# mpetri/ans-large-alphabet

Measured on AMD Instinct MI355X. Metric: encode+decode Mints/s (uint32), bit-exact vs CPU reference per block, higher is better.
Workload: dtype u32 symbols; ANS state carried as an exact f64 (integers below 2^53) in the encoder, u64 in the decoder; 1 GPU; ANSfold-1 on 268435456 uint32 per GPU, zipf20s1.2, blocks of 16384 ints, restart every 1024; codec=ANSfold-1, ints_per_gpu=268435456, distribution=zipf20s1.2, block_ints=16384, ckpt_interval=1024, seed=1234, multi_gpu=single GPU

## Files before the change

ans_large_alphabet_amd/csrc/ansx.hip:

```cpp
#include "../../include/ansx.h"

#include <hip/hip_runtime.h>
#include <dlfcn.h>
#include <rccl/rccl.h>

#include <algorithm>
#include <array>
#include <cmath>
#include <cstdio>
#include <cstdlib>
#include <cstring>
#include <deque>
#include <functional>
#include <map>
#include <set>
#include <string>
#include <vector>

#include "ansx_kernels.h"
#include "ansx_rfold.h"
#include "ansx_model.h"
#include "ansx_fastmodel.h"
#include "ansx_gen.h"
#include "ansx_pa.h"
#include "ansx_intsparse.h"
#include "ansx_ranges.h"
#include "ansx_batch.h"

namespace {

struct DevBuf {
    void* p = nullptr;
    size_t cap = 0;
};

struct ProfRec {
    std::string name;
    hipEvent_t e0, e1;
};

struct Layout {
    u64 index_off, ckoff_off, ckstate_off, hint_off, payload_off;
};

}

struct ansx_ctx {
    u32 num_cus = 256;
    int device = 0;
    hipStream_t stream = nullptr;
    int last_hip = 0;
    bool profile = false;
    std::vector<ProfRec> recs;
    std::map<std::string, std::pair<double, u64>> acc;
    std::vector<std::string> order;
    DevBuf pre_work;
    DevBuf hist, hterm, sortF, sortSym, attS, prevS, attMeta, blk, table, tab32, scratch, misc, mapped, mostfreq,
        stage_in, stage_out, dec_s2s, dec_cum, dec_info, plain, rf_tmp, log2lut, pa_alpha, pa_info, pairs, lg2i, sizes, nearlist, force;
    DevBuf rng_plan, rng_cont, rng_list;
    DevBuf rng_dev;
    DevBuf bat_hdr;
    u8* rng_pin = nullptr;
    size_t rng_pin_cap = 0;
    u32* h_pin = nullptr;
    std::map<u64, u32> ns_hint;
    std::map<u64, u32> rf_hint;
    std::map<std::array<u64, 4>, ansx_container_header> hdr_cache;
    std::deque<std::array<u64, 4>> hdr_order;
    std::map<u32, DevBuf> geo;
    DevBuf geo_big;
    u32 geo_big_cap = 0;
    int last_gather_ranks = 0;
    std::set<u64> wide_hint;
    std::map<u64, u32> t_hint;
    const u32* cur_force = nullptr;
    const u32* cur_src = nullptr;
    bool used_pc = false;
    bool used_fast = false;
    u32 cur_nt = 0;
    u32 cur_rf_slots = 0;
    u32 cur_pa_distinct = 0;
    std::set<u64> int_sparse_hint;
    bool cur_int_sparse = false;
    u32 sp_retries = 0;
    bool sp_full_lds = false;
    ansx_encode_stats last = {};
    struct {
        bool table16_fixup = false;
        bool encode_gtab16 = false;
        bool parse_generic = false;
        bool parse_win = false;
        bool parse_fast = false;
        bool decode_table = false;
        bool no_stream_lds = false;
        int decode_mode = 0;
        u32 parse_stage_words = 0;
        bool model_fused = false;
        bool model_sync = false;
        bool use_pc = false;
        u32 pc_b_pairs = 2;
        u32 test_sp_bits = 0;
        bool fin_one_wave = false;
        bool no_big_geo = false;
        bool no_pc_auto = false;
        bool encode_mode2 = false;
        bool force_pc = false;
        bool no_pc = false;
        int decode_small_ring = 0;
        int decode_pair = 0;
        u32 pair_lds_limit = 0;
        u32 wide_at = 16;
        bool wide_restart = false;
        u32 ns_hint = 0;
        u32 t_hint = 0;
        bool no_fast_model = false;
        double near_band = ANSX_NEAR_BAND;
        bool near_flip = false;
        u32 cand_chains = 0;
        double fast_guard = ANSX_FAST_GUARD;
        u32 batch_pass_blocks = 0;
    } dbg;
};

namespace {

#define HIPCHK(ctx, call)                                                                        \
    do {                                                                                         \
        hipError_t _e = (call);                                                                  \
        if (_e != hipSuccess) {                                                                  \
            (ctx)->last_hip = (int)_e;                                                           \
            return ANSX_ERR_HIP;                                                                 \
        }                                                                                        \
    } while (0)

int ensure(ansx_ctx* c, DevBuf& b, size_t bytes)
{
    if (bytes <= b.cap) return ANSX_OK;
    if (b.p) {
        hipError_t e = hipFree(b.p);
        b.p = nullptr;
        b.cap = 0;
        if (e != hipSuccess) {
// ... 16 lines not shown
    if (!c->profile) return;
    ProfRec r;
    r.name = name;
    (void)hipEventCreate(&r.e0);
    (void)hipEventCreate(&r.e1);
    (void)hipEventRecord(r.e0, s);
    c->recs.push_back(r);
}
void prof_end(ansx_ctx* c, hipStream_t s)
{
    if (!c->profile) return;
    (void)hipEventRecord(c->recs.back().e1, s);
}

#define LAUNCH(ctx, name, kern, grid, block, shmem, strm, ...)                                   \
    do {                                                                                         \
        prof_begin(ctx, name, strm);                                                             \
        hipLaunchKernelGGL(kern, dim3(grid), dim3(block), (shmem), strm, __VA_ARGS__);           \
        prof_end(ctx, strm);                                                                     \
        HIPCHK(ctx, hipGetLastError());                                                          \
    } while (0)

inline size_t rup(size_t v, size_t a) { return (v + a - 1) / a * a; }

size_t codec_nsp(int kind, u32 f) { return kind == ANSX_MSB ? 2048u : (kind == ANSX_INT ? 16384u : fold_NSP(f)); }

size_t block_bound(int kind, u32 f, size_t nb, bool pa = false)
{
    size_t hdr = kind == ANSX_RFOLD ? 4 + 4 * (size_t)fold_T(f) : 0;
    size_t nsp = codec_nsp(kind, f);
    if (pa) hdr += 8 + 4 * nb + 8;
    return hdr + 8 + 4 * nsp + 7 * nb + 32;
}

struct Plan {
    ansx_geo g;
    bool plain;
    Layout lay;
    u32 NSP;
    const ansx_blk_out* bout = nullptr;
    u64 bout_ints = 0;
};

Layout layout_of(const ansx_geo& g, bool plain)
{
    Layout L;
// ... 355 lines not shown
        && !c->dbg.encode_gtab16 && (u64)scr_stride * 16 < 0x7FFFFF00ull;
    c->used_fast = fast;
    if (fast && NSP > 4096 && !c->dbg.no_big_geo) {
        if (c->geo_big_cap < fcap_probe) {
            if ((rc = ensure(c, c->geo_big, ((size_t)fcap_probe * (fcap_probe + 1) / 2 + 8) * 8))) return rc;
            LAUNCH(c, "k_build_interp_geo", k_build_interp_geo, fcap_probe, 256, 0, s, fcap_probe, (uint2*)c->geo_big.p);
            c->geo_big_cap = fcap_probe;
        }
        geo = (const uint2*)c->geo_big.p;
    }
    if (fast) {
        if ((rc = ensure(c, c->pairs, (size_t)NB * NSP * 8))) return rc;
        if (!c->lg2i.p) {
            if ((rc = ensure(c, c->lg2i, (size_t)65536 * 8))) return rc;
            LAUNCH(c, "k_build_log2i_lut", k_build_log2i_lut, 256, 256, 0, s, (double*)c->lg2i.p);
        }
    }
    double* hterm = nullptr;
    if (h_deferred && !h_in_hist && !fast) {
        if ((rc = ensure(c, c->hterm, (size_t)NB * NSP * 8))) return rc;
        hterm = (double*)c->hterm.p;
    }
    const size_t hist_lds = !h_in_hist ? (size_t)NSP * 4 : (size_t)4 * (NSP + ANSX_HCOPY_PAD) * 4 + (fast ? 0 : (size_t)NSP * 8 + 80);
    if (NSP >= 8192u) {
        const size_t packed_lds = (size_t)NSP * 2;
        if (packed_lds > 48 * 1024)
            HIPCHK(c, hipFuncSetAttribute((const void*)k_fold_hist<true>, hipFuncAttributeMaxDynamicSharedMemorySize, (int)packed_lds));
        LAUNCH(c, "k_fold_hist", k_fold_hist<true>, (size_t)NB * cpb, 256, packed_lds, s, src, g, chunk, cpb, NSP, hist, hterm,
            fast ? 2u : 0u, blk, gflags, (g.kind == ANSX_INT && !g.pa) ? NSP : (1u << 30));
    } else {
        if (hist_lds > 48 * 1024)
            HIPCHK(c, hipFuncSetAttribute((const void*)k_fold_hist<false>, hipFuncAttributeMaxDynamicSharedMemorySize, (int)hist_lds));
        LAUNCH(c, "k_fold_hist", k_fold_hist<false>, (size_t)NB * cpb, 256, hist_lds, s, src, g, chunk, cpb, NSP, hist, hterm,
            (h_in_hist ? 1u : 0u) | (fast ? 2u : 0u), blk, gflags, (g.kind == ANSX_INT && !g.pa) ? NSP : (1u << 30));
    }
    const u32 nbig_cap = (u32)std::min<size_t>(NSP, (size_t)g.block_ints / ANSX_VMAX + 2);
    const u32 sort_cap = (optimistic && h_deferred) ? std::min<u32>(NSP, std::max<u32>(64u, (ns_cap + 7u) & ~7u)) : NSP;
    const bool sort16 = g.block_ints <= 65535u;
    size_t k2a_lds = (size_t)nbig_cap * 8 + (size_t)sort_cap * (sort16 ? 2 : 4) + (h_deferred ? 0 : 512 * 8);
    const bool sort_staged = k2a_lds <= 150 * 1024;
    if (!sort_staged) k2a_lds = (size_t)nbig_cap * 8 + (h_deferred ? 0 : 512 * 8);
    if (k2a_lds > 32 * 1024) {
        HIPCHK(c, hipFuncSetAttribute((const void*)k_sort_entropy<u16>, hipFuncAttributeMaxDynamicSharedMemorySize, (int)k2a_lds));
        HIPCHK(c, hipFuncSetAttribute((const void*)k_sort_entropy<u32>, hipFuncAttributeMaxDynamicSharedMemorySize, (int)k2a_lds));
    }
    if ((size_t)NSP * 8 + 64 > 48 * 1024 && (size_t)NSP * 8 + 64 <= 150 * 1024)
        HIPCHK(c, hipFuncSetAttribute((const void*)k_write_prelude<0>,
                      hipFuncAttributeMaxDynamicSharedMemorySize, (int)((size_t)NSP * 8 + 64)));
    if (!sort_staged)
        LAUNCH(c, "k_sort_entropy", (k_sort_entropy<u32, false>), NB, 64, k2a_lds, s, g, NSP, nbig_cap, h_deferred ? 1u : 0u, hist,
            (u32*)c->sortF.p, (u16*)c->sortSym.p, blk, sort_cap, fast ? (uint2*)c->pairs.p : (uint2*)nullptr, gflags);
    else if (sort16)
        LAUNCH(c, "k_sort_entropy", k_sort_entropy<u16>, NB, 64, k2a_lds, s, g, NSP, nbig_cap, h_deferred ? 1u : 0u, hist,
            (u32*)c->sortF.p, (u16*)c->sortSym.p, blk, sort_cap, fast ? (uint2*)c->pairs.p : (uint2*)nullptr, gflags);
    else
        LAUNCH(c, "k_sort_entropy", k_sort_entropy<u32>, NB, 64, k2a_lds, s, g, NSP, nbig_cap, h_deferred ? 1u : 0u, hist,
            (u32*)c->sortF.p, (u16*)c->sortSym.p, blk, sort_cap, fast ? (uint2*)c->pairs.p : (uint2*)nullptr, gflags);
    const u32 nbatch = 24 / ANSX_ATTEMPTS;
    u32 max_logM = 0, max_ns = 0;
    const bool test_fixup = c->dbg.table16_fixup;
    const u32 always16 = (!test_fixup && (NSP > 4096 || (u64)scr_stride * 16 >= 0x7FFFFF00ull || c->dbg.encode_gtab16)) ? 1u : 0u;
    u32* hints = (P.plain || (g.kind == ANSX_INT && !g.pa)) ? nullptr : (u32*)(d_out + P.lay.hint_off);
    if (fast) {
        const u32 bpw = 64u / NT;
        const u32 nch = c->dbg.cand_chains ? c->dbg.cand_chains : (((NB + bpw - 1) / bpw <= 4u * c->num_cus) ? 1u : 2u);
        const size_t cl = (size_t)ANSX_CAND_WAVES * nch * bpw * ANSX_CAND_ROW * 16;
        const u32 cwaves = (NB + nch * bpw - 1) / (nch * bpw);
#define ANSX_LAUNCH_CAND2(NT_, NCH_)                                                                                    \
    do {                                                                                                            \
        if (cl > 48 * 1024)                                                                                         \
            HIPCHK(c, hipFuncSetAttribute((const void*)k_candidates<NT_, NCH_>, hipFuncAttributeMaxDynamicSharedMemorySize, (int)cl)); \
        LAUNCH(c, "k_candidates", (k_candidates<NT_, NCH_>), (cwaves + ANSX_CAND_WAVES - 1) / ANSX_CAND_WAVES, 64 * ANSX_CAND_WAVES, cl, s, g, NSP, \
            (const uint2*)c->pairs.p, (const ansx_blk*)blk, (uint4*)c->attS.p, (u32*)c->attMeta.p);               \
    } while (0)
#define ANSX_LAUNCH_CAND(NT_)                                                                                           \
    do {                                                                                                            \
        if (nch == 1) ANSX_LAUNCH_CAND2(NT_, 1);                                                                    \
        else ANSX_LAUNCH_CAND2(NT_, 2);                                                                             \
    } while (0)
        switch (NT) {
        case 4: ANSX_LAUNCH_CAND(4); break;
        case 5: ANSX_LAUNCH_CAND(5); break;
        case 6: ANSX_LAUNCH_CAND(6); break;
        case 7: ANSX_LAUNCH_CAND(7); break;
        default: ANSX_LAUNCH_CAND(8); break;
        }
#undef ANSX_LAUNCH_CAND
#undef ANSX_LAUNCH_CAND2
        const u32 fcap = std::min<u32>(NSP, std::max<u32>(64u, (ns_cap + 15u) & ~15u));
        const bool fin_generic = NSP > 4096;
        const size_t fl = (size_t)fcap * (fin_generic ? 8 : 12) + 64;
#define ANSX_LAUNCH_FIN(IPT_, NTC_)                                                                                    \
    do {                                                                                                            \
        if (fl > 48 * 1024)                                                                                         \
            HIPCHK(c, hipFuncSetAttribute((const void*)k_model_finish<IPT_, NTC_>, hipFuncAttributeMaxDynamicSharedMemorySize, (int)fl)); \
        LAUNCH(c, "k_model_finish", (k_model_finish<IPT_, NTC_>), NB, 256, fl, s, g, NSP, NT, (const uint2*)c->pairs.p, (const uint4*)c->attS.p, \
            (const u32*)c->attMeta.p, blk, (u32*)c->tab32.p, (u8*)c->scratch.p, (u64)scr_stride, mostfreq, hints, gflags, fcap, c->dbg.fast_guard, (const double*)c->lg2i.p, geo, \
            fin_generic ? hist : (u32*)nullptr); \
    } while (0)
        if (NSP <= 1024 && c->dbg.fin_one_wave) {
            if (NT <= 5) {
                LAUNCH(c, "k_model_finish", (k_model_finish<16, 5, 64>), NB, 64, fl, s, g, NSP, NT, (const uint2*)c->pairs.p, (const uint4*)c->attS.p,
                    (const u32*)c->attMeta.p, blk, (u32*)c->tab32.p, (u8*)c->scratch.p, (u64)scr_stride, mostfreq, hints, gflags, fcap, c->dbg.fast_guard, (const double*)c->lg2i.p, geo,
                    (u32*)nullptr);
            } else {
                LAUNCH(c, "k_model_finish", (k_model_finish<16, 8, 64>), NB, 64, fl, s, g, NSP, NT, (const uint2*)c->pairs.p, (const uint4*)c->attS.p,
                    (const u32*)c->attMeta.p, blk, (u32*)c->tab32.p, (u8*)c->scratch.p, (u64)scr_stride, mostfreq, hints, gflags, fcap, c->dbg.fast_guard, (const double*)c->lg2i.p, geo,
                    (u32*)nullptr);
            }
        } else if (NSP <= 1024) {
            ANSX_LAUNCH_FIN(4, 8);
        } else if (NSP > 4096) {
            if (NT <= 5) ANSX_LAUNCH_FIN(0, 5);
            else ANSX_LAUNCH_FIN(0, 8);
        } else {
            if (NT <= 5) ANSX_LAUNCH_FIN(16, 5);
            else ANSX_LAUNCH_FIN(16, 8);
        }
#undef ANSX_LAUNCH_FIN
        max_logM = 16;
        max_ns = ns_cap;
    }
    for (u32 batch = 0; batch < (fast ? 0u : nbatch); batch++) {
        if (batch) HIPCHK(c, hipMemsetAsync(&gflags[ANSX_G_PAD], 0, 4, s));
        LAUNCH(c, "k_scale_attempts", k_scale_attempts, ((size_t)NB * ANSX_ATTEMPTS + 255) / 256, 256,
            0, s, g, NSP, batch, hist, (const u32*)c->sortF.p, (const u16*)c->sortSym.p, blk,
            (u16*)c->attS.p, (u32*)c->attMeta.p, (const double*)hterm, (const ansx_log2_ent*)c->log2lut.p,
            g.block_ints <= 65535u ? 1u : 0u);
        LAUNCH(c, "k_select_model", k_select_model, NB, 64, 0, s, g, NSP, batch, hist,
            (const u16*)c->attS.p, (const u32*)c->attMeta.p, (u16*)c->prevS.p, blk,
            (ansx_enc_entry*)c->table.p, (u32*)c->tab32.p, gflags, batch == nbatch - 1 ? 1u : 0u, always16,
            (u32*)c->nearlist.p, c->cur_force, c->dbg.near_band, c->dbg.near_flip ? 1u : 0u);
        if (optimistic) {
            max_logM = 16;
            max_ns = ns_cap;
            break;
        }
        HIPCHK(c, hipMemcpyAsync(c->h_pin, c->misc.p, 16, hipMemcpyDeviceToHost, s));
        HIPCHK(c, hipStreamSynchronize(s));
        int st0 = flags_to_status(c->h_pin[ANSX_G_ERR]);
        if (st0) return st0;
        max_logM = c->h_pin[ANSX_G_MAXLOGM];
// ... 1251 lines not shown
    if (hipGetDeviceCount(&ndev) != hipSuccess || ndev == 0) return ANSX_ERR_NO_DEVICE;
    if (device < 0) {
        if (hipGetDevice(&device) != hipSuccess) return ANSX_ERR_NO_DEVICE;
    }
    if (device >= ndev) return ANSX_ERR_ARG;
    if (hipSetDevice(device) != hipSuccess) return ANSX_ERR_NO_DEVICE;
    hipDeviceProp_t prop;
    if (hipGetDeviceProperties(&prop, device) != hipSuccess) return ANSX_ERR_NO_DEVICE;
    if (strncmp(prop.gcnArchName, "gfx950", 6) != 0) return ANSX_ERR_NO_DEVICE;
    ansx_ctx* c = new ansx_ctx();
    c->device = device;
    c->num_cus = prop.multiProcessorCount > 0 ? (u32)prop.multiProcessorCount : 256u;
    if (hipStreamCreateWithFlags(&c->stream, hipStreamDefault) != hipSuccess) {
        delete c;
        return ANSX_ERR_HIP;
    }
    if (hipHostMalloc((void**)&c->h_pin, 4096, hipHostMallocDefault) != hipSuccess) {
        (void)hipStreamDestroy(c->stream);
        delete c;
        return ANSX_ERR_HIP;
    }
    static const char* const names[] = { "ANSX_TEST_TABLE16_FIXUP", "ANSX_ENCODE_GTAB16", "ANSX_PARSE_GENERIC", "ANSX_PARSE_WIN", "ANSX_PARSE_FAST",
        "ANSX_DECODE_TABLE", "ANSX_NO_STREAM_LDS", "ANSX_DECODE_MODE", "ANSX_PARSE_STAGE_WORDS", "ANSX_MODEL_FUSED", "ANSX_MODEL_SYNC", "ANSX_NS_HINT", "ANSX_T_HINT", "ANSX_NO_FAST_MODEL", "ANSX_FAST_GUARD", "ANSX_CAND_CHAINS", "ANSX_NEAR_BAND", "ANSX_TEST_NEAR_FLIP", "ANSX_WIDE_RESTART", "ANSX_TEST_WIDE_AT",
        "ANSX_BATCH_PASS_BLOCKS" };
    for (const char* nm : names)
        if (const char* v = getenv(nm)) (void)ansx_debug_set(c, nm, v);
    *out = c;
    return ANSX_OK;
}

int ansx_last_encode_stats(const ansx_ctx* c, ansx_encode_stats* out)
{
    if (!c || !out) return ANSX_ERR_ARG;
    *out = c->last;
#ifdef ANSX_STAMPS
    {
        static unsigned long long h[16 * 256 + 16];
        if (hipMemcpyFromSymbol(h, HIP_SYMBOL(g_stamps), sizeof(h)) == hipSuccess) {
            double acc[16] = {};
            int nn = 0;
#ifdef ANSX_STAMPS_RF
            const int last = 8;
#else
            const int last = 10;
#endif
            for (int w = 0; w < 256; w++) {
                if (!h[w * 16] || !h[w * 16 + last]) continue;
// ... 57 lines not shown
    else if (!strcmp(name, "ANSX_PC_B_PAIRS")) c->dbg.pc_b_pairs = (value && value[0] == '1') ? 1u : 2u;
    else if (!strcmp(name, "ANSX_ENCODE_MODE2")) c->dbg.encode_mode2 = on;
    else if (!strcmp(name, "ANSX_DECODE_SMALL_RING"))
        c->dbg.decode_small_ring = !value ? 0 : !strcmp(value, "never") ? 1 : !strcmp(value, "always") ? 2 : 0;
    else if (!strcmp(name, "ANSX_DECODE_PAIR"))
        c->dbg.decode_pair = !value ? 0 : !strcmp(value, "never") ? 1 : !strcmp(value, "always") ? 2 : 0;
    else if (!strcmp(name, "ANSX_DECODE_PAIR_LDS")) c->dbg.pair_lds_limit = (value && value[0]) ? (u32)strtoul(value, nullptr, 10) : 0u;
    else if (!strcmp(name, "ANSX_FORGET_HINTS")) {
        c->ns_hint.clear();
        c->rf_hint.clear();
        c->t_hint.clear();
        c->wide_hint.clear();
        c->hdr_cache.clear();
        c->hdr_order.clear();
    }
    else if (!strcmp(name, "ANSX_TEST_WIDE_AT")) {
        const u32 v = (value && value[0]) ? (u32)strtoul(value, nullptr, 10) : 16u;
        if (v > 16) return ANSX_ERR_ARG;
        c->dbg.wide_at = v;
    }
    else if (!strcmp(name, "ANSX_NEAR_BAND")) c->dbg.near_band = (value && value[0]) ? strtod(value, nullptr) : ANSX_NEAR_BAND;
    else if (!strcmp(name, "ANSX_TEST_NEAR_FLIP")) c->dbg.near_flip = on;
    else if (!strcmp(name, "ANSX_BATCH_PASS_BLOCKS")) c->dbg.batch_pass_blocks = (value && value[0]) ? (u32)strtoul(value, nullptr, 10) : 0u;
    else if (!strcmp(name, "ANSX_CAND_CHAINS")) {
        const u32 v = value ? (u32)strtoul(value, nullptr, 10) : 0u;
        if (v > 2) return ANSX_ERR_ARG;
        c->dbg.cand_chains = v;
    } else if (!strcmp(name, "ANSX_FAST_GUARD")) c->dbg.fast_guard = (value && value[0]) ? strtod(value, nullptr) : ANSX_FAST_GUARD;
    else return ANSX_ERR_ARG;
    return ANSX_OK;
}

void ansx_destroy(ansx_ctx* c)
{
    if (!c) return;
    (void)hipSetDevice(c->device);
    (void)hipStreamSynchronize(c->stream);
    DevBuf* bufs[] = { &c->pre_work, &c->hist, &c->hterm, &c->sortF, &c->sortSym, &c->attS, &c->prevS, &c->attMeta, &c->blk,
        &c->table, &c->tab32, &c->scratch, &c->misc, &c->mapped, &c->mostfreq, &c->stage_in, &c->stage_out,
        &c->dec_s2s, &c->dec_cum, &c->dec_info, &c->plain, &c->rf_tmp, &c->log2lut, &c->pa_alpha, &c->pa_info, &c->pairs, &c->lg2i, &c->sizes, &c->nearlist, &c->force, &c->geo_big,
        &c->rng_plan, &c->rng_cont, &c->rng_list, &c->rng_dev, &c->bat_hdr };
    for (DevBuf* b : bufs)
        if (b->p) (void)hipFree(b->p);
    for (auto& kv : c->geo)
        if (kv.second.p) (void)hipFree(kv.second.p);
    for (auto& r : c->recs) {
        (void)hipEventDestroy(r.e0);
        (void)hipEventDestroy(r.e1);
    }
    if (c->h_pin) (void)hipHostFree(c->h_pin);
    if (c->rng_pin) (void)hipHostFree(c->rng_pin);
    (void)hipStreamDestroy(c->stream);
    delete c;
}

const char* ansx_strerror(int st)
{
    switch (st) {
    case ANSX_OK: return "ok";
    case ANSX_ERR_ARG: return "invalid argument";
// ... 460 lines not shown
```

ans_large_alphabet_amd/csrc/ansx_fastmodel.h:

```cpp
#pragma once

#include "ansx_kernels.h"

#ifdef ANSX_STAMPS_RF
#undef STAMP
#define STAMP(i) do { } while (0)
#endif

#define ANSX_FAST_GUARD 1e-9
#define ANSX_CAND_SL 64u
#define ANSX_CAND_ROW (ANSX_CAND_SL + 1u)
#define ANSX_CAND_MAXBPW 16u
#define ANSX_FIN_LUT 512u

__global__ void k_build_log2i_lut(double* __restrict__ lut)
{
    const u32 i = blockIdx.x * 256 + threadIdx.x;
    if (i < 65536u) lut[i] = i ? ansx_log2_portable((double)i) : 0.0;
}

__device__ __forceinline__ double ansx_rcp_int31(double b)
{
    const double y0 = __builtin_amdgcn_rcp(b);
    const double y1 = __builtin_fma(__builtin_fma(-b, y0, 1.0), y0, y0);
    return __builtin_fma(__builtin_fma(-b, y1, 1.0), y1, y1);
}

ANSX_HD u64 srank_chunk(u32 NSP, u32 NT, u32 b, u32 batch, u32 t) { return ((u64)b * (NSP / 8u) + batch) * NT + t; }

#define ANSX_CAND_WAVES 4u
template <u32 NT, u32 NCH>
__global__ __launch_bounds__(64 * ANSX_CAND_WAVES) void k_candidates(ansx_geo g, u32 NSP,
    const uint2* __restrict__ pairs, const ansx_blk* __restrict__ blk, uint4* __restrict__ srank,
    u32* __restrict__ attMeta)
{
    extern __shared__ double2 cand_lds_all[];
    const u32 lane = threadIdx.x & 63u, wv = threadIdx.x >> 6;
    constexpr u32 BPW = 64u / NT;
    constexpr u32 rows = NCH * BPW;
    double2* const cand_lds = cand_lds_all + wv * rows * ANSX_CAND_ROW;
    const u32 bl = lane / NT, t = lane - bl * NT;
    const u32 wb0 = (u32)__builtin_amdgcn_readfirstlane((int)((blockIdx.x * ANSX_CAND_WAVES + wv) * rows));
    if (wb0 >= g.nblocks) return;
    u32 bb[NCH], sigma[NCH], sh[NCH];
    bool live[NCH];
    double Md[NCH], fsd[NCH], mx[NCH];
    uint4* sp[NCH];
    const double2* row[NCH];
    u32 wsig = 0;
#pragma unroll
    for (u32 c = 0; c < NCH; c++) {
        bb[c] = wb0 + c * BPW + bl;
        live[c] = bl < BPW && bb[c] < g.nblocks;
        sigma[c] = 0, sh[c] = 0;
        double nd = 1.0;
        if (live[c]) {
            const ansx_blk* B = &blk[bb[c]];
            sigma[c] = B->sigma;
            sh[c] = B->m0_log2 + t;
            nd = (double)B->n;
        }
        wsig = sigma[c] > wsig ? sigma[c] : wsig;
        const bool dead = sh[c] > 31;
        Md[c] = dead ? -1.0 : (double)((u64)1 << (dead ? 0u : sh[c]));
        fsd[c] = nd;
        mx[c] = 0.0;
        sp[c] = srank + srank_chunk(NSP, NT, live[c] ? bb[c] : wb0, 0u, t);
        row[c] = cand_lds + (c * BPW + (bl < BPW ? bl : BPW - 1u)) * ANSX_CAND_ROW;
    }
    wsig = wave_max(wsig);
    constexpr u32 NITER = rows * (ANSX_CAND_SL / 64u);
    uint2 nxt[NITER];
    const u32 last_b = g.nblocks - 1u;
    auto fetch = [&](u32 c0) {
#pragma unroll
        for (u32 k = 0; k < NITER; k++) {
            const u32 i = k * 64u + lane;
            u32 b2 = wb0 + i / ANSX_CAND_SL;
            b2 = b2 < last_b ? b2 : last_b;
            u32 j = c0 + (i % ANSX_CAND_SL);
            j = j < NSP ? j : NSP - 1u;
            nxt[k] = pairs[(u64)b2 * NSP + j];
        }
    };
    auto commit = [&]() {
#pragma unroll
        for (u32 k = 0; k < NITER; k++) {
            const u32 i = k * 64u + lane;
            const u32 rem = nxt[k].y ? nxt[k].y : 1u;
            cand_lds[(i / ANSX_CAND_SL) * ANSX_CAND_ROW + (i % ANSX_CAND_SL)] =
                double2{ (double)(nxt[k].x & 0xFFFFu), ansx_rcp_int31((double)rem) };
        }
    };
    auto step = [&](u32 c, const double2 e) -> u32 {
        const double q = Md[c] * e.y;
        const double r = __builtin_fma(-q, fsd[c], Md[c]);
// ... 95 lines not shown
#ifdef ANSX_STAMPS
        t_loop += wall_clock64() - t_a;
#endif
    }
#ifdef ANSX_STAMPS
    if (threadIdx.x == 0 && blockIdx.x < 256) {
        g_stamps[blockIdx.x * 16 + 12] = t_commit;
        g_stamps[blockIdx.x * 16 + 13] = t_loop;
        g_stamps[blockIdx.x * 16 + 14] = wall_clock64() - tc0;
    }
#endif
#pragma unroll
    for (u32 c = 0; c < NCH; c++)
        if (live[c])
            *(uint2*)(attMeta + ((u64)bb[c] * ANSX_ATTEMPTS + t) * 4) =
                make_uint2((Md[c] == 0.0) ? 1u : 0u, mx[c] >= 4294967295.0 ? 0xFFFFFFFFu : (u32)mx[c]);
}

template <int IPT, int NTC, int NTH = 256>
__global__ __launch_bounds__(NTH) void k_model_finish(ansx_geo g, u32 NSP, u32 NT, const uint2* __restrict__ pairs,
    const uint4* __restrict__ srank, const u32* __restrict__ attMeta, ansx_blk* __restrict__ blk,
    u32* __restrict__ tab32, u8* __restrict__ scratch, u64 scr_stride, const u32* __restrict__ mostfreq,
    u32* __restrict__ hints, u32* __restrict__ gflags, u32 cap, double guard, const double* __restrict__ lg2i,
    const uint2* __restrict__ geo, u32* __restrict__ incbuf = nullptr)
{
    static_assert(IPT % 4 == 0, "table rows are written 16 bytes at a time");
    static_assert(ANSX_FIN_LUT == 512 && (NTH == 256 || NTH == 64), "two table entries per thread (eight in the one-wave form)");
    static_assert(NTH == 256 || (IPT > 4), "the one-wave form takes every candidate in every lane");
    static_assert(NTC >= 4 && NTC <= (int)ANSX_ATTEMPTS, "candidates per block");
    extern __shared__ u32 lds32[];
    __shared__ u32 sh_part[8];
    __shared__ double lut[ANSX_FIN_LUT];
    __shared__ double wpart[ANSX_ATTEMPTS][4];
    __shared__ double wsum[ANSX_ATTEMPTS];
    const u32 tid = threadIdx.x, lane = tid & 63u, wv = tid >> 6;
    const u32 b = blockIdx.x;
    ansx_blk* B = &blk[b];
    u32* off = lds32;
    u32* bits = lds32 + cap;
    const bool inc_hbm = IPT == 0 && incbuf != nullptr;
    u32* inc = inc_hbm ? incbuf + (u64)b * NSP : lds32 + 2 * cap;
    const u32 dump = inc_hbm ? cap + 8u : 2u * cap + 8u;
    u32* frq = bits;
    STAMP(0);
    const u32 ns = B->max_sym + 1;
    const u32 sigma = B->sigma;
    const double thr = B->thr;
    const u32 m0 = B->m0_log2;
    const double nd = (double)B->n;
    uint2 mt[ANSX_ATTEMPTS];
#pragma unroll
    for (u32 t = 0; t < ANSX_ATTEMPTS; t++) mt[t] = t < NT ? *(const uint2*)(attMeta + ((u64)b * ANSX_ATTEMPTS + t) * 4) : make_uint2(0u, 0u);
    double2 l2[256 / NTH];
#pragma unroll
    for (int i = 0; i < 256 / NTH; i++) l2[i] = *(const double2*)(lg2i + 2 * (tid + NTH * i));
    const uint2* prow = pairs + (u64)b * NSP;
    auto load_fs = [&](u32 c, u32 (&fs)[8]) {
        const uint2* pp = prow + (u64)c * 8u;
        const uint4 a0 = *(const uint4*)pp, a1 = *(const uint4*)(pp + 2), a2 = *(const uint4*)(pp + 4), a3 = *(const uint4*)(pp + 6);
// ... 243 lines not shown
```

ans_large_alphabet_amd/csrc/ansx_kernels.h:

```cpp
#pragma once

#include <type_traits>

#include "ansx_dev.h"

#ifdef ANSX_STAMPS
__device__ unsigned long long g_stamps[16 * 256 + 16];
#define STAMP(i) do { if (threadIdx.x == 0 && blockIdx.x % 61 == 7 && blockIdx.x / 61 < 256) g_stamps[(blockIdx.x / 61) * 16 + (i)] = wall_clock64(); } while (0)
#else
#define STAMP(i) do { } while (0)
#endif
#ifdef ANSX_STAMPS_RF
#define STAMP_RF(i) STAMP(i)
#else
#define STAMP_RF(i) do { } while (0)
#endif

struct ansx_blk {
    u32 n;
    u32 max_sym;
    u32 sigma;
    u32 m0_log2;
    double H;
    double thr;
// ... 39 lines not shown
struct ansx_zero4 {
    uint4* p[4];
    u64 n16[4];
};
__global__ __launch_bounds__(256) void k_begin_encode(ansx_zero4 Z)
{
    const u64 stride = (u64)gridDim.x * 256;
    const uint4 z = make_uint4(0u, 0u, 0u, 0u);
#pragma unroll
    for (int r = 0; r < 4; r++)
        for (u64 i = (u64)blockIdx.x * 256 + threadIdx.x; i < Z.n16[r]; i += stride) Z.p[r][i] = z;
}

#define ANSX_HCOPY_PAD 8u
typedef u32 ansx_u32x4 __attribute__((ext_vector_type(4)));
__device__ __forceinline__ uint4 ld16_stream(const uint4* p)
{
    const ansx_u32x4 v = __builtin_nontemporal_load((const ansx_u32x4*)p);
    return make_uint4(v.x, v.y, v.z, v.w);
}
template <bool PACKED>
__global__ __launch_bounds__(256) void k_fold_hist(const u32* __restrict__ in, ansx_geo g,
    u32 chunk, u32 cpb, u32 NSP, u32* __restrict__ hist, double* __restrict__ hterm, u32 sum_mode,
    ansx_blk* __restrict__ blk, u32* __restrict__ gflags, u32 value_limit)
{
    const u32 sum_here = sum_mode & 1u;
    const bool tree_sum = (sum_mode & 2u) != 0;
    extern __shared__ u32 lds_hist[];
    const u32 tid = threadIdx.x;
    const u32 b = blockIdx.x / cpb, c = blockIdx.x % cpb;
    const u32 nb = geo_block_n(g, b);
    const u64 start = (u64)c * chunk;
    if (start >= nb) return;
    const u32 len = (u32)((nb - start) < chunk ? (nb - start) : chunk);
    const u32* src = in + (u64)b * g.block_ints + start;
    const u32 cstride = sum_here ? NSP + ANSX_HCOPY_PAD : 0;
    const u32 hwords = sum_here ? 4 * cstride : (PACKED ? NSP / 2 : NSP);
    auto hcount = [&](u32 sy) -> u32 {
        if constexpr (PACKED) return (lds_hist[sy >> 1] >> (16u * (sy & 1u))) & 0xFFFFu;
        else return lds_hist[sy];
    };
    for (u32 s = tid; s < hwords; s += 256) lds_hist[s] = 0;
    u32* const aux = lds_hist + hwords;
    if (sum_here && !tree_sum && tid < 17) aux[2 * NSP + tid] = 0;
    u32* const my_hist = lds_hist + (tid & 3) * cstride;
    __syncthreads();
    const ansx_map mp = g.map;
    const bool ident = g.kind == 3;
    u32 lmax = 0, bad = 0;
    auto take = [&](u32 x) {
        bad |= (x >= value_limit) ? 1u : 0u;
        u32 k = map_nbytes(mp, x);
        u32 s = map_sym(mp, x, k);
// ... 98 lines not shown
        }
    } else {
        for (u32 s = tid; s < NSP; s += 256) {
            u32 v = hcount(s);
            if (v) atomicAdd(&h[s], v);
        }
    }
    lmax = wave_max(lmax);
    bad = wave_or(bad);
    if ((tid & 63) == 0) {
        atomicMax(&blk[b].max_sym, lmax);
        if (bad) atomicOr(&gflags[ANSX_G_ERR], 1u << 6 );
    }
}

#define ANSX_VMAX 256u
#define ANSX_MASKV 256u

__device__ __forceinline__ void wave_lds_sync() { asm volatile("s_waitcnt lgkmcnt(0)" ::: "memory"); }

template <typename HT, bool STAGED = true>
__global__ __launch_bounds__(64) void k_sort_entropy(ansx_geo g, u32 NSP, u32 nbig_cap, u32 h_deferred,
    const u32* __restrict__ hist, u32* __restrict__ sortF, u16* __restrict__ sortSym,
    ansx_blk* __restrict__ blk, u32 cap, uint2* __restrict__ pairs, u32* __restrict__ gflags)
{
    extern __shared__ u64 lds_k2a[];
    __shared__ u32 cnt[ANSX_VMAX];
    __shared__ u16 cnt0[ANSX_VMAX];
    __shared__ unsigned long long vmask[ANSX_MASKV];
    __shared__ u32 wadj[ANSX_VMAX];
    __shared__ u32 sh_nbig;
    u64* big_keys = lds_k2a;
    HT* hrow = (HT*)(lds_k2a + nbig_cap);
    double* terms = (double*)(hrow + (STAGED ? cap : 0u));
    const u32 lane = threadIdx.x;
    const u32 b = blockIdx.x;
    const u32* h = hist + (u64)b * NSP;
    constexpr u32 SORT_PRE = 10;
    u32 hp[SORT_PRE];
#pragma unroll
    for (u32 r = 0; r < SORT_PRE; r++) hp[r] = r * 64 + lane < NSP ? h[r * 64 + lane] : 0u;
    const u32 ns = blk[b].max_sym + 1;
    auto hget = [&](u32 sy) -> u32 {
        if constexpr (STAGED) return hrow[sy];
        else return h[sy];
    };
    if (STAGED && ns > cap) {
        if (lane == 0) {
            blk[b].status = 9;
            blk[b].resolved = 1;
            atomicOr(&gflags[ANSX_G_ERR], 1u << ANSX_G_VIOL_BIT);
        }
        return;
    }
    u32* oF = sortF + (u64)b * NSP;
    u16* oS = sortSym + (u64)b * NSP;
    uint2* oP = pairs ? pairs + (u64)b * NSP : nullptr;
    if constexpr (STAGED) {
#pragma unroll
// ... 3614 lines not shown
```

Baseline: 140,800 Mints/s.

## Pipeline model-building kernels over block ranges on side streams

Splits the per-block model stages (histogram, sort/entropy, candidates, finish) into two block ranges. The histogram for the next range runs on the main stream while sort, candidates and finish for the previous range run on alternating non-blocking side streams, joined back with events. The aim is to overlap the memory-bound histogram pass with the compute-heavy model kernels. It adds stream and event management, range-bounded kernel indexing, and a default trigger for large inputs (NB≥8192 blocks and ≥2^27 ints). The trigger is skipped during graph capture or profiling.

```diff
diff --git a/ans_large_alphabet_amd/csrc/ansx.hip b/ans_large_alphabet_amd/csrc/ansx.hip
--- a/ans_large_alphabet_amd/csrc/ansx.hip
+++ b/ans_large_alphabet_amd/csrc/ansx.hip
@@ -44,6 +44,13 @@
 };
 
 }
+
+#define ANSX_PIPE_NEVER (-1)
+#define ANSX_PIPE_ALWAYS (-2)
+#define ANSX_PIPE_MAX_RANGES 64
+#define ANSX_PIPE_RANGES 2u
+#define ANSX_PIPE_MIN_BLOCKS 8192u
+#define ANSX_PIPE_MIN_INTS ((u64)1 << 27)
 
 struct ansx_ctx {
     u32 num_cus = 256;
@@ -85,6 +92,8 @@
     u32 sp_retries = 0;
     bool sp_full_lds = false;
     ansx_encode_stats last = {};
+    hipStream_t pipe_stream[2] = { nullptr, nullptr };
+    std::vector<hipEvent_t> pipe_ev;
     struct {
         bool table16_fixup = false;
         bool encode_gtab16 = false;
@@ -118,6 +127,7 @@
         bool near_flip = false;
         u32 cand_chains = 0;
         double fast_guard = ANSX_FAST_GUARD;
+        int model_pipeline = 0;
         u32 batch_pass_blocks = 0;
     } dbg;
 };
@@ -180,6 +190,24 @@
     } while (0)
 
 inline size_t rup(size_t v, size_t a) { return (v + a - 1) / a * a; }
+
+int pipe_hip(ansx_ctx* c, hipError_t e)
+{
+    if (e == hipSuccess) return ANSX_OK;
+    c->last_hip = (int)e;
+    return ANSX_ERR_HIP;
+}
+int pipeline_prepare(ansx_ctx* c, u32 nranges)
+{
+    for (hipStream_t& st : c->pipe_stream)
+        if (!st) HIPCHK(c, hipStreamCreateWithFlags(&st, hipStreamNonBlocking));
+    while (c->pipe_ev.size() < 2 + (size_t)nranges) {
+        hipEvent_t e;
+        HIPCHK(c, hipEventCreateWithFlags(&e, hipEventDisableTiming));
+        c->pipe_ev.push_back(e);
+    }
+    return ANSX_OK;
+}
 
 size_t codec_nsp(int kind, u32 f) { return kind == ANSX_MSB ? 2048u : (kind == ANSX_INT ? 16384u : fold_NSP(f)); }
 
@@ -581,57 +609,108 @@
         hterm = (double*)c->hterm.p;
     }
     const size_t hist_lds = !h_in_hist ? (size_t)NSP * 4 : (size_t)4 * (NSP + ANSX_HCOPY_PAD) * 4 + (fast ? 0 : (size_t)NSP * 8 + 80);
-    if (NSP >= 8192u) {
-        const size_t packed_lds = (size_t)NSP * 2;
-        if (packed_lds > 48 * 1024)
-            HIPCHK(c, hipFuncSetAttribute((const void*)k_fold_hist<true>, hipFuncAttributeMaxDynamicSharedMemorySize, (int)packed_lds));
-        LAUNCH(c, "k_fold_hist", k_fold_hist<true>, (size_t)NB * cpb, 256, packed_lds, s, src, g, chunk, cpb, NSP, hist, hterm,
-            fast ? 2u : 0u, blk, gflags, (g.kind == ANSX_INT && !g.pa) ? NSP : (1u << 30));
-    } else {
-        if (hist_lds > 48 * 1024)
-            HIPCHK(c, hipFuncSetAttribute((const void*)k_fold_hist<false>, hipFuncAttributeMaxDynamicSharedMemorySize, (int)hist_lds));
-        LAUNCH(c, "k_fold_hist", k_fold_hist<false>, (size_t)NB * cpb, 256, hist_lds, s, src, g, chunk, cpb, NSP, hist, hterm,
-            (h_in_hist ? 1u : 0u) | (fast ? 2u : 0u), blk, gflags, (g.kind == ANSX_INT && !g.pa) ? NSP : (1u << 30));
-    }
     const u32 nbig_cap = (u32)std::min<size_t>(NSP, (size_t)g.block_ints / ANSX_VMAX + 2);
     const u32 sort_cap = (optimistic && h_deferred) ? std::min<u32>(NSP, std::max<u32>(64u, (ns_cap + 7u) & ~7u)) : NSP;
     const bool sort16 = g.block_ints <= 65535u;
     size_t k2a_lds = (size_t)nbig_cap * 8 + (size_t)sort_cap * (sort16 ? 2 : 4) + (h_deferred ? 0 : 512 * 8);
     const bool sort_staged = k2a_lds <= 150 * 1024;
     if (!sort_staged) k2a_lds = (size_t)nbig_cap * 8 + (h_deferred ? 0 : 512 * 8);
-    if (k2a_lds > 32 * 1024) {
-        HIPCHK(c, hipFuncSetAttribute((const void*)k_sort_entropy<u16>, hipFuncAttributeMaxDynamicSharedMemorySize, (int)k2a_lds));
-        HIPCHK(c, hipFuncSetAttribute((const void*)k_sort_entropy<u32>, hipFuncAttributeMaxDynamicSharedMemorySize, (int)k2a_lds));
-    }
-    if ((size_t)NSP * 8 + 64 > 48 * 1024 && (size_t)NSP * 8 + 64 <= 150 * 1024)
-        HIPCHK(c, hipFuncSetAttribute((const void*)k_write_prelude<0>,
-                      hipFuncAttributeMaxDynamicSharedMemorySize, (int)((size_t)NSP * 8 + 64)));
-    if (!sort_staged)
-        LAUNCH(c, "k_sort_entropy", (k_sort_entropy<u32, false>), NB, 64, k2a_lds, s, g, NSP, nbig_cap, h_deferred ? 1u : 0u, hist,
-            (u32*)c->sortF.p, (u16*)c->sortSym.p, blk, sort_cap, fast ? (uint2*)c->pairs.p : (uint2*)nullptr, gflags);
-    else if (sort16)
-        LAUNCH(c, "k_sort_entropy", k_sort_entropy<u16>, NB, 64, k2a_lds, s, g, NSP, nbig_cap, h_deferred ? 1u : 0u, hist,
-            (u32*)c->sortF.p, (u16*)c->sortSym.p, blk, sort_cap, fast ? (uint2*)c->pairs.p : (uint2*)nullptr, gflags);
-    else
-        LAUNCH(c, "k_sort_entropy", k_sort_entropy<u32>, NB, 64, k2a_lds, s, g, NSP, nbig_cap, h_deferred ? 1u : 0u, hist,
-            (u32*)c->sortF.p, (u16*)c->sortSym.p, blk, sort_cap, fast ? (uint2*)c->pairs.p : (uint2*)nullptr, gflags);
     const u32 nbatch = 24 / ANSX_ATTEMPTS;
     u32 max_logM = 0, max_ns = 0;
     const bool test_fixup = c->dbg.table16_fixup;
     const u32 always16 = (!test_fixup && (NSP > 4096 || (u64)scr_stride * 16 >= 0x7FFFFF00ull || c->dbg.encode_gtab16)) ? 1u : 0u;
     u32* hints = (P.plain || (g.kind == ANSX_INT && !g.pa)) ? nullptr : (u32*)(d_out + P.lay.hint_off);
+    const u32 bpw = fast ? 64u / NT : 1u;
+    auto cand_chains = [&](u32 nblk) -> u32 {
+        return c->dbg.cand_chains ? c->dbg.cand_chains : (((nblk + bpw - 1) / bpw <= 4u * c->num_cus) ? 1u : 2u);
+    };
+    const u32 fcap = std::min<u32>(NSP, std::max<u32>(64u, (ns_cap + 15u) & ~15u));
+    const bool fin_generic = NSP > 4096;
+    const size_t fl = (size_t)fcap * (fin_generic ? 8 : 12) + 64;
+
+    u32 range_blocks = NB, nranges = 0;
+    if (fast && !c->profile && c->dbg.model_pipeline != ANSX_PIPE_NEVER) {
+        const int mode = c->dbg.model_pipeline;
+        u32 want = mode > 0 ? (u32)mode : ((mode == ANSX_PIPE_ALWAYS || (NB >= ANSX_PIPE_MIN_BLOCKS && g.n >= ANSX_PIPE_MIN_INTS)) ? ANSX_PIPE_RANGES : 0u);
+        if (want) {
+            hipStreamCaptureStatus cs = hipStreamCaptureStatusNone;
+            if (hipStreamIsCapturing(s, &cs) != hipSuccess || cs != hipStreamCaptureStatusNone) want = 0;
+        }
+        if (want) {
+            range_blocks = (u32)rup(((size_t)NB + want - 1) / want, 64);
+            nranges = (NB + range_blocks - 1) / range_blocks;
+            if ((rc = pipeline_prepare(c, nranges))) return rc;
+        }
+    }
+
+    const bool hist_packed = NSP >= 8192u;
+    const size_t packed_lds = (size_t)NSP * 2;
+    if (hist_packed) {
+        if (packed_lds > 48 * 1024)
+            HIPCHK(c, hipFuncSetAttribute((const void*)k_fold_hist<true>, hipFuncAttributeMaxDynamicSharedMemorySize, (int)packed_lds));
+    } else if (hist_lds > 48 * 1024)
+        HIPCHK(c, hipFuncSetAttribute((const void*)k_fold_hist<false>, hipFuncAttributeMaxDynamicSharedMemorySize, (int)hist_lds));
+    if (k2a_lds > 32 * 1024) {
+        HIPCHK(c, hipFuncSetAttribute((const void*)k_sort_entropy<u16>, hipFuncAttributeMaxDynamicSharedMemorySize, (int)k2a_lds));
+        HIPCHK(c, hipFuncSetAttribute((const void*)k_sort_entropy<u32>, hipFuncAttributeMaxDynamicSharedMemorySize, (int)k2a_lds));
+    }
+    if ((size_t)NSP * 8 + 64 > 48 * 1024 && (size_t)NSP * 8 + 64 <= 150 * 1024)
+        HIPCHK(c, hipFuncSetAttribute((const void*)k_write_prelude<0>,
+                      hipFuncAttributeMaxDynamicSharedMemorySize, (int)((size_t)NSP * 8 + 64)));
     if (fast) {
-        const u32 bpw = 64u / NT;
-        const u32 nch = c->dbg.cand_chains ? c->dbg.cand_chains : (((NB + bpw - 1) / bpw <= 4u * c->num_cus) ? 1u : 2u);
+        const u32 last_blocks = nranges ? NB - (nranges - 1) * range_blocks : NB;
+        const u32 chain_set = (1u << cand_chains(nranges ? range_blocks : NB)) | (1u << cand_chains(last_blocks));
+        for (u32 nch = 1; nch <= 2; nch++) {
+            const size_t cl = (size_t)ANSX_CAND_WAVES * nch * bpw * ANSX_CAND_ROW * 16;
+            if (!(chain_set & (1u << nch)) || cl <= 48 * 1024) continue;
+            const void* fn = nullptr;
+            switch (NT) {
+            case 4: fn = nch == 1 ? (const void*)k_candidates<4, 1> : (const void*)k_candidates<4, 2>; break;
+            case 5: fn = nch == 1 ? (const void*)k_candidates<5, 1> : (const void*)k_candidates<5, 2>; break;
+            case 6: fn = nch == 1 ? (const void*)k_candidates<6, 1> : (const void*)k_candidates<6, 2>; break;
+            case 7: fn = nch == 1 ? (const void*)k_candidates<7, 1> : (const void*)k_candidates<7, 2>; break;
+            default: fn = nch == 1 ? (const void*)k_candidates<8, 1> : (const void*)k_candidates<8, 2>; break;
+            }
+            HIPCHK(c, hipFuncSetAttribute(fn, hipFuncAttributeMaxDynamicSharedMemorySize, (int)cl));
+        }
+        if (fl > 48 * 1024 && !(NSP <= 1024 && c->dbg.fin_one_wave)) {
+            const void* fn = NSP <= 1024 ? (const void*)k_model_finish<4, 8>
+                : NSP > 4096 ? (NT <= 5 ? (const void*)k_model_finish<0, 5> : (const void*)k_model_finish<0, 8>)
+                             : (NT <= 5 ? (const void*)k_model_finish<16, 5> : (const void*)k_model_finish<16, 8>);
+            HIPCHK(c, hipFuncSetAttribute(fn, hipFuncAttributeMaxDynamicSharedMemorySize, (int)fl));
+        }
+    }
+
+    auto launch_hist = [&](hipStream_t st, u32 b0, u32 be) -> int {
+        const size_t grid = (size_t)(be - b0) * cpb;
+        if (hist_packed) {
+            LAUNCH(c, "k_fold_hist", k_fold_hist<true>, grid, 256, packed_lds, st, src, g, chunk, cpb, NSP, hist, hterm,
+                fast ? 2u : 0u, blk, gflags, (g.kind == ANSX_INT && !g.pa) ? NSP : (1u << 30), b0, be);
+        } else {
+            LAUNCH(c, "k_fold_hist", k_fold_hist<false>, grid, 256, hist_lds, st, src, g, chunk, cpb, NSP, hist, hterm,
+                (h_in_hist ? 1u : 0u) | (fast ? 2u : 0u), blk, gflags, (g.kind == ANSX_INT && !g.pa) ? NSP : (1u << 30), b0, be);
+        }
+        return ANSX_OK;
+    };
+    auto launch_sort = [&](hipStream_t st, u32 b0, u32 be) -> int {
+        if (!sort_staged)
+            LAUNCH(c, "k_sort_entropy", (k_sort_entropy<u32, false>), be - b0, 64, k2a_lds, st, g, NSP, nbig_cap, h_deferred ? 1u : 0u, hist,
+                (u32*)c->sortF.p, (u16*)c->sortSym.p, blk, sort_cap, fast ? (uint2*)c->pairs.p : (uint2*)nullptr, gflags, b0, be);
+        else if (sort16)
+            LAUNCH(c, "k_sort_entropy", k_sort_entropy<u16>, be - b0, 64, k2a_lds, st, g, NSP, nbig_cap, h_deferred ? 1u : 0u, hist,
+                (u32*)c->sortF.p, (u16*)c->sortSym.p, blk, sort_cap, fast ? (uint2*)c->pairs.p : (uint2*)nullptr, gflags, b0, be);
+        else
+            LAUNCH(c, "k_sort_entropy", k_sort_entropy<u32>, be - b0, 64, k2a_lds, st, g, NSP, nbig_cap, h_deferred ? 1u : 0u, hist,
+                (u32*)c->sortF.p, (u16*)c->sortSym.p, blk, sort_cap, fast ? (uint2*)c->pairs.p : (uint2*)nullptr, gflags, b0, be);
+        return ANSX_OK;
+    };
+    auto launch_cand = [&](hipStream_t st, u32 b0, u32 be) -> int {
+        const u32 nch = cand_chains(be - b0);
         const size_t cl = (size_t)ANSX_CAND_WAVES * nch * bpw * ANSX_CAND_ROW * 16;
-        const u32 cwaves = (NB + nch * bpw - 1) / (nch * bpw);
+        const u32 cwaves = (be - b0 + nch * bpw - 1) / (nch * bpw);
 #define ANSX_LAUNCH_CAND2(NT_, NCH_)                                                                                    \
-    do {                                                                                                            \
-        if (cl > 48 * 1024)                                                                                         \
-            HIPCHK(c, hipFuncSetAttribute((const void*)k_candidates<NT_, NCH_>, hipFuncAttributeMaxDynamicSharedMemorySize, (int)cl)); \
-        LAUNCH(c, "k_candidates", (k_candidates<NT_, NCH_>), (cwaves + ANSX_CAND_WAVES - 1) / ANSX_CAND_WAVES, 64 * ANSX_CAND_WAVES, cl, s, g, NSP, \
-            (const uint2*)c->pairs.p, (const ansx_blk*)blk, (uint4*)c->attS.p, (u32*)c->attMeta.p);               \
-    } while (0)
+        LAUNCH(c, "k_candidates", (k_candidates<NT_, NCH_>), (cwaves + ANSX_CAND_WAVES - 1) / ANSX_CAND_WAVES, 64 * ANSX_CAND_WAVES, cl, st, g, NSP, \
+            (const uint2*)c->pairs.p, (const ansx_blk*)blk, (uint4*)c->attS.p, (u32*)c->attMeta.p, b0, be)
 #define ANSX_LAUNCH_CAND(NT_)                                                                                           \
     do {                                                                                                            \
         if (nch == 1) ANSX_LAUNCH_CAND2(NT_, 1);                                                                    \
@@ -646,37 +725,65 @@
         }
 #undef ANSX_LAUNCH_CAND
 #undef ANSX_LAUNCH_CAND2
-        const u32 fcap = std::min<u32>(NSP, std::max<u32>(64u, (ns_cap + 15u) & ~15u));
-        const bool fin_generic = NSP > 4096;
-        const size_t fl = (size_t)fcap * (fin_generic ? 8 : 12) + 64;
-#define ANSX_LAUNCH_FIN(IPT_, NTC_)                                                                                    \
-    do {                                                                                                            \
-        if (fl > 48 * 1024)                                                                                         \
-            HIPCHK(c, hipFuncSetAttribute((const void*)k_model_finish<IPT_, NTC_>, hipFuncAttributeMaxDynamicSharedMemorySize, (int)fl)); \
-        LAUNCH(c, "k_model_finish", (k_model_finish<IPT_, NTC_>), NB, 256, fl, s, g, NSP, NT, (const uint2*)c->pairs.p, (const uint4*)c->attS.p, \
+        return ANSX_OK;
+    };
+    auto launch_fin = [&](hipStream_t st, u32 b0, u32 be) -> int {
+#define ANSX_LAUNCH_FIN(IPT_, NTC_, NTH_)                                                                              \
+        LAUNCH(c, "k_model_finish", (k_model_finish<IPT_, NTC_, NTH_>), be - b0, NTH_, fl, st, g, NSP, NT, (const uint2*)c->pairs.p, (const uint4*)c->attS.p, \
             (const u32*)c->attMeta.p, blk, (u32*)c->tab32.p, (u8*)c->scratch.p, (u64)scr_stride, mostfreq, hints, gflags, fcap, c->dbg.fast_guard, (const double*)c->lg2i.p, geo, \
-            fin_generic ? hist : (u32*)nullptr); \
-    } while (0)
+            (fin_generic && (NTH_) == 256) ? hist : (u32*)nullptr, b0, be)
         if (NSP <= 1024 && c->dbg.fin_one_wave) {
-            if (NT <= 5) {
-                LAUNCH(c, "k_model_finish", (k_model_finish<16, 5, 64>), NB, 64, fl, s, g, NSP, NT, (const uint2*)c->pairs.p, (const uint4*)c->attS.p,
-                    (const u32*)c->attMeta.p, blk, (u32*)c->tab32.p, (u8*)c->scratch.p, (u64)scr_stride, mostfreq, hints, gflags, fcap, c->dbg.fast_guard, (const double*)c->lg2i.p, geo,
-                    (u32*)nullptr);
-            } else {
-                LAUNCH(c, "k_model_finish", (k_model_finish<16, 8, 64>), NB, 64, fl, s, g, NSP, NT, (const uint2*)c->pairs.p, (const uint4*)c->attS.p,
-                    (const u32*)c->attMeta.p, blk, (u32*)c->tab32.p, (u8*)c->scratch.p, (u64)scr_stride, mostfreq, hints, gflags, fcap, c->dbg.fast_guard, (const double*)c->lg2i.p, geo,
-                    (u32*)nullptr);
+            if (NT <= 5) ANSX_LAUNCH_FIN(16, 5, 64);
+            else ANSX_LAUNCH_FIN(16, 8, 64);
+        } else if (NSP <= 1024) {
+            ANSX_LAUNCH_FIN(4, 8, 256);
+        } else if (NSP > 4096) {
+            if (NT <= 5) ANSX_LAUNCH_FIN(0, 5, 256);
+            else ANSX_LAUNCH_FIN(0, 8, 256);
+        } else {
+            if (NT <= 5) ANSX_LAUNCH_FIN(16, 5, 256);
+            else ANSX_LAUNCH_FIN(16, 8, 256);
+        }
+#undef ANSX_LAUNCH_FIN
+        return ANSX_OK;
+    };
+    if (nranges == 0) {
+        if ((rc = launch_hist(s, 0, NB))) return rc;
+        if ((rc = launch_sort(s, 0, NB))) return rc;
+        if (fast) {
+            if ((rc = launch_cand(s, 0, NB))) return rc;
+            if ((rc = launch_fin(s, 0, NB))) return rc;
+        }
+    } else {
+        u32 used = 0;
+        rc = ANSX_OK;
+        for (u32 k = 0; k < nranges && !rc; k++) {
+            const u32 b0 = k * range_blocks, be = std::min<u32>(NB, b0 + range_blocks);
+            if ((rc = launch_hist(s, b0, be))) break;
+            hipStream_t st = s;
+            if (k + 1 < nranges) {
+                const u32 side = k & 1u;
+                st = c->pipe_stream[side];
+                if ((rc = pipe_hip(c, hipEventRecord(c->pipe_ev[2 + k], s)))) break;
+                if ((rc = pipe_hip(c, hipStreamWaitEvent(st, c->pipe_ev[2 + k], 0)))) break;
+                used |= 1u << side;
             }
-        } else if (NSP <= 1024) {
-            ANSX_LAUNCH_FIN(4, 8);
-        } else if (NSP > 4096) {
-            if (NT <= 5) ANSX_LAUNCH_FIN(0, 5);
-            else ANSX_LAUNCH_FIN(0, 8);
-        } else {
-            if (NT <= 5) ANSX_LAUNCH_FIN(16, 5);
-            else ANSX_LAUNCH_FIN(16, 8);
-        }
-#undef ANSX_LAUNCH_FIN
+            if ((rc = launch_sort(st, b0, be))) break;
+            if ((rc = launch_cand(st, b0, be))) break;
+            rc = launch_fin(st, b0, be);
+        }
+        for (u32 side = 0; side < 2; side++) {
+            if (!(used & (1u << side))) continue;
+            int rj = pipe_hip(c, hipEventRecord(c->pipe_ev[side], c->pipe_stream[side]));
+            if (!rj) rj = pipe_hip(c, hipStreamWaitEvent(s, c->pipe_ev[side], 0));
+            if (rj) {
+                (void)hipStreamSynchronize(c->pipe_stream[side]);
+                if (!rc) rc = rj;
+            }
+        }
+        if (rc) return rc;
+    }
+    if (fast) {
         max_logM = 16;
         max_ns = ns_cap;
     }
@@ -1974,7 +2081,7 @@
     }
     static const char* const names[] = { "ANSX_TEST_TABLE16_FIXUP", "ANSX_ENCODE_GTAB16", "ANSX_PARSE_GENERIC", "ANSX_PARSE_WIN", "ANSX_PARSE_FAST",
         "ANSX_DECODE_TABLE", "ANSX_NO_STREAM_LDS", "ANSX_DECODE_MODE", "ANSX_PARSE_STAGE_WORDS", "ANSX_MODEL_FUSED", "ANSX_MODEL_SYNC", "ANSX_NS_HINT", "ANSX_T_HINT", "ANSX_NO_FAST_MODEL", "ANSX_FAST_GUARD", "ANSX_CAND_CHAINS", "ANSX_NEAR_BAND", "ANSX_TEST_NEAR_FLIP", "ANSX_WIDE_RESTART", "ANSX_TEST_WIDE_AT",
-        "ANSX_BATCH_PASS_BLOCKS" };
+        "ANSX_BATCH_PASS_BLOCKS", "ANSX_MODEL_PIPELINE" };
     for (const char* nm : names)
         if (const char* v = getenv(nm)) (void)ansx_debug_set(c, nm, v);
     *out = c;
@@ -2078,6 +2185,17 @@
     else if (!strcmp(name, "ANSX_NEAR_BAND")) c->dbg.near_band = (value && value[0]) ? strtod(value, nullptr) : ANSX_NEAR_BAND;
     else if (!strcmp(name, "ANSX_TEST_NEAR_FLIP")) c->dbg.near_flip = on;
     else if (!strcmp(name, "ANSX_BATCH_PASS_BLOCKS")) c->dbg.batch_pass_blocks = (value && value[0]) ? (u32)strtoul(value, nullptr, 10) : 0u;
+    else if (!strcmp(name, "ANSX_MODEL_PIPELINE")) {
+        if (!value || !value[0] || !strcmp(value, "0")) c->dbg.model_pipeline = 0;
+        else if (!strcmp(value, "never")) c->dbg.model_pipeline = ANSX_PIPE_NEVER;
+        else if (!strcmp(value, "always")) c->dbg.model_pipeline = ANSX_PIPE_ALWAYS;
+        else {
+            char* end = nullptr;
+            const unsigned long v = strtoul(value, &end, 10);
+            if (value[0] < '0' || value[0] > '9' || *end != 0 || v < 1 || v > ANSX_PIPE_MAX_RANGES) return ANSX_ERR_ARG;
+            c->dbg.model_pipeline = (int)v;
+        }
+    }
     else if (!strcmp(name, "ANSX_CAND_CHAINS")) {
         const u32 v = value ? (u32)strtoul(value, nullptr, 10) : 0u;
         if (v > 2) return ANSX_ERR_ARG;
@@ -2092,6 +2210,11 @@
     if (!c) return;
     (void)hipSetDevice(c->device);
     (void)hipStreamSynchronize(c->stream);
+    for (hipStream_t st : c->pipe_stream)
+        if (st) (void)hipStreamSynchronize(st);
+    for (hipEvent_t e : c->pipe_ev) (void)hipEventDestroy(e);
+    for (hipStream_t st : c->pipe_stream)
+        if (st) (void)hipStreamDestroy(st);
     DevBuf* bufs[] = { &c->pre_work, &c->hist, &c->hterm, &c->sortF, &c->sortSym, &c->attS, &c->prevS, &c->attMeta, &c->blk,
         &c->table, &c->tab32, &c->scratch, &c->misc, &c->mapped, &c->mostfreq, &c->stage_in, &c->stage_out,
         &c->dec_s2s, &c->dec_cum, &c->dec_info, &c->plain, &c->rf_tmp, &c->log2lut, &c->pa_alpha, &c->pa_info, &c->pairs, &c->lg2i, &c->sizes, &c->nearlist, &c->force, &c->geo_big,
diff --git a/ans_large_alphabet_amd/csrc/ansx_fastmodel.h b/ans_large_alphabet_amd/csrc/ansx_fastmodel.h
--- a/ans_large_alphabet_amd/csrc/ansx_fastmodel.h
+++ b/ans_large_alphabet_amd/csrc/ansx_fastmodel.h
@@ -32,16 +32,17 @@
 template <u32 NT, u32 NCH>
 __global__ __launch_bounds__(64 * ANSX_CAND_WAVES) void k_candidates(ansx_geo g, u32 NSP,
     const uint2* __restrict__ pairs, const ansx_blk* __restrict__ blk, uint4* __restrict__ srank,
-    u32* __restrict__ attMeta)
+    u32* __restrict__ attMeta, u32 b0, u32 bend)
 {
+
     extern __shared__ double2 cand_lds_all[];
     const u32 lane = threadIdx.x & 63u, wv = threadIdx.x >> 6;
     constexpr u32 BPW = 64u / NT;
     constexpr u32 rows = NCH * BPW;
     double2* const cand_lds = cand_lds_all + wv * rows * ANSX_CAND_ROW;
     const u32 bl = lane / NT, t = lane - bl * NT;
-    const u32 wb0 = (u32)__builtin_amdgcn_readfirstlane((int)((blockIdx.x * ANSX_CAND_WAVES + wv) * rows));
-    if (wb0 >= g.nblocks) return;
+    const u32 wb0 = (u32)__builtin_amdgcn_readfirstlane((int)(b0 + (blockIdx.x * ANSX_CAND_WAVES + wv) * rows));
+    if (wb0 >= bend) return;
     u32 bb[NCH], sigma[NCH], sh[NCH];
     bool live[NCH];
     double Md[NCH], fsd[NCH], mx[NCH];
@@ -51,7 +52,7 @@
 #pragma unroll
     for (u32 c = 0; c < NCH; c++) {
         bb[c] = wb0 + c * BPW + bl;
-        live[c] = bl < BPW && bb[c] < g.nblocks;
+        live[c] = bl < BPW && bb[c] < bend;
         sigma[c] = 0, sh[c] = 0;
         double nd = 1.0;
         if (live[c]) {
@@ -71,7 +72,7 @@
     wsig = wave_max(wsig);
     constexpr u32 NITER = rows * (ANSX_CAND_SL / 64u);
     uint2 nxt[NITER];
-    const u32 last_b = g.nblocks - 1u;
+    const u32 last_b = bend - 1u;
     auto fetch = [&](u32 c0) {
 #pragma unroll
         for (u32 k = 0; k < NITER; k++) {
@@ -213,7 +214,7 @@
     const uint4* __restrict__ srank, const u32* __restrict__ attMeta, ansx_blk* __restrict__ blk,
     u32* __restrict__ tab32, u8* __restrict__ scratch, u64 scr_stride, const u32* __restrict__ mostfreq,
     u32* __restrict__ hints, u32* __restrict__ gflags, u32 cap, double guard, const double* __restrict__ lg2i,
-    const uint2* __restrict__ geo, u32* __restrict__ incbuf = nullptr)
+    const uint2* __restrict__ geo, u32* __restrict__ incbuf, u32 b0, u32 bend)
 {
     static_assert(IPT % 4 == 0, "table rows are written 16 bytes at a time");
     static_assert(ANSX_FIN_LUT == 512 && (NTH == 256 || NTH == 64), "two table entries per thread (eight in the one-wave form)");
@@ -225,7 +226,8 @@
     __shared__ double wpart[ANSX_ATTEMPTS][4];
     __shared__ double wsum[ANSX_ATTEMPTS];
     const u32 tid = threadIdx.x, lane = tid & 63u, wv = tid >> 6;
-    const u32 b = blockIdx.x;
+    const u32 b = b0 + blockIdx.x;
+    if (b >= bend) return;
     ansx_blk* B = &blk[b];
     u32* off = lds32;
     u32* bits = lds32 + cap;
diff --git a/ans_large_alphabet_amd/csrc/ansx_kernels.h b/ans_large_alphabet_amd/csrc/ansx_kernels.h
--- a/ans_large_alphabet_amd/csrc/ansx_kernels.h
+++ b/ans_large_alphabet_amd/csrc/ansx_kernels.h
@@ -85,13 +85,14 @@
 template <bool PACKED>
 __global__ __launch_bounds__(256) void k_fold_hist(const u32* __restrict__ in, ansx_geo g,
     u32 chunk, u32 cpb, u32 NSP, u32* __restrict__ hist, double* __restrict__ hterm, u32 sum_mode,
-    ansx_blk* __restrict__ blk, u32* __restrict__ gflags, u32 value_limit)
+    ansx_blk* __restrict__ blk, u32* __restrict__ gflags, u32 value_limit, u32 b0, u32 bend)
 {
     const u32 sum_here = sum_mode & 1u;
     const bool tree_sum = (sum_mode & 2u) != 0;
     extern __shared__ u32 lds_hist[];
     const u32 tid = threadIdx.x;
-    const u32 b = blockIdx.x / cpb, c = blockIdx.x % cpb;
+    const u32 b = b0 + blockIdx.x / cpb, c = blockIdx.x % cpb;
+    if (b >= bend) return;
     const u32 nb = geo_block_n(g, b);
     const u64 start = (u64)c * chunk;
     if (start >= nb) return;
@@ -236,7 +237,7 @@
 template <typename HT, bool STAGED = true>
 __global__ __launch_bounds__(64) void k_sort_entropy(ansx_geo g, u32 NSP, u32 nbig_cap, u32 h_deferred,
     const u32* __restrict__ hist, u32* __restrict__ sortF, u16* __restrict__ sortSym,
-    ansx_blk* __restrict__ blk, u32 cap, uint2* __restrict__ pairs, u32* __restrict__ gflags)
+    ansx_blk* __restrict__ blk, u32 cap, uint2* __restrict__ pairs, u32* __restrict__ gflags, u32 b0, u32 bend)
 {
     extern __shared__ u64 lds_k2a[];
     __shared__ u32 cnt[ANSX_VMAX];
@@ -248,7 +249,8 @@
     HT* hrow = (HT*)(lds_k2a + nbig_cap);
     double* terms = (double*)(hrow + (STAGED ? cap : 0u));
     const u32 lane = threadIdx.x;
-    const u32 b = blockIdx.x;
+    const u32 b = b0 + blockIdx.x;
+    if (b >= bend) return;
     const u32* h = hist + (u64)b * NSP;
     constexpr u32 SORT_PRE = 10;
     u32 hp[SORT_PRE];
```

Measured after the change: 146,300 Mints/s (median of 6 runs). 1.04x the previous value.
